# mfathulkr/MA-CJD-Cooperative-Jamming-Decision-Making-via-MARL

Measured on AMD Instinct MI355X. Metric: env-steps/sec (all GPUs; batch_envs=4096/GPU, 3j/4r), higher is better.
Workload: dtype f64; 1 GPU; 3 jammers / 4 radars, batch_envs=4096 per GPU, GRU hidden=64; mode=train, hidden=64, train_batch_episodes=32, updates_per_graph=20, hip_graphs=True, gemm_tuning=True, update=paired: Q-head launches as one grid, mixers as one grid, the chain on one queue, replay_capacity_episodes=8192, mixer_dtype=fp32, mixer=one MFMA launch per direction (f32)

## Files before the change

### include/macjd_nets.h

```cpp
#ifndef MACJD_NETS_H
#define MACJD_NETS_H

#include <stdint.h>

#ifdef __cplusplus
extern "C" {
#endif

typedef struct macjd_qhead_io {
    int64_t n_rows;
    int32_t H, A, n_agents, greedy_only;
    const float* base;  int64_t base_ld;
    const float* P_all; int64_t p_ld;
    const float* W1;    int64_t w1_ld;
    const float* w2;
    const float* b2;
    float* Q;           int64_t q_ld;
    const void* avail;  int32_t avail_elem_size, reserved;
    int64_t av_se, av_sj, av_sa;
    float epsilon;      float reserved2;
    uint64_t seed, counter;
    const float* eps_dev;
    const uint64_t* counter_dev;
    int32_t* T_out32;
// ... 234 lines not shown
    float* sn; float* xhat;
    float* act;
    const float* gy;
    float* gq;
    float* gout1;
    float* g_w1raw;
    float* g_wfraw;
    float* g_v;
} macjd_mixerf_io;

int macjd_mixer_fused_supported(int32_t J, int32_t S, int32_t Hh, int32_t Em);
int macjd_mixer_fused_forward(const macjd_mixerf_io* io, void* hip_stream);
int macjd_mixer_fused_forward_pair(const macjd_mixerf_io* saved, const macjd_mixerf_io* plain, void* hip_stream);
int macjd_mixer_fused_backward(const macjd_mixerf_io* io, void* hip_stream);
int macjd_mixer_fused_backward_td(const macjd_mixerf_io* io, const macjd_tdloss_io* td, const float* tot_m, void* hip_stream);

typedef struct macjd_agent_episode_io {
    int64_t n_envs;
    int32_t T, J, H, A;
    int32_t greedy_only, reserved;
    const float* gi;    int64_t gi_ld;
    const float* P_all; int64_t p_ld;
    const float* h0;
    const float* w_hh;  const float* b_hh;
    const float* W1;    int64_t w1_ld;
    const float* b1;    const float* w2; const float* b2;
    const void* avail;  int32_t avail_elem_size, reserved2;
    int64_t av_se, av_sj, av_sa;
    const float* eps;
    uint64_t seed;
// ... 31 lines not shown
```

### ma-cjd-cooperative-jamming-decision-making-via-marl_amd/_native.py

```python
from __future__ import annotations

import ctypes
import os
from typing import Optional

_PKG_DIR = os.path.dirname(os.path.abspath(__file__))
LIB_NAME = "libmacjd_hip.so"
LIB_PATH = os.environ.get("MACJD_LIB") or os.path.join(_PKG_DIR, LIB_NAME)

ABI_VERSION = 3
STEP_ARITH_F64 = 1
STEP_LANE_KERNEL = 2
STEP_SLOT_KERNEL = 4

EXPORTS = [
    "macjd_abi_version", "macjd_last_error", "macjd_reload_options", "macjd_device_count",
    "macjd_scenario_create", "macjd_scenario_destroy", "macjd_scenario_dims", "macjd_scenario_is_regular",
    "macjd_env_reset", "macjd_env_step", "macjd_env_step_timed",
    "macjd_qhead_select", "macjd_gru_sequence", "macjd_mixer_tail_forward", "macjd_mixer_tail_backward",
    "macjd_mlp_forward", "macjd_mlp_forward_pair", "macjd_td_loss", "macjd_clip_adam_step", "macjd_clip_adam_step_sample", "macjd_clip_adam_step_ln", "macjd_sample_episodes", "macjd_gather_rows",
    "macjd_linear_wgrad", "macjd_linear_wgrad_workspace_floats", "macjd_linear_wgrad_many", "macjd_qhead_input", "macjd_layernorm_forward", "macjd_layernorm_param_grad", "macjd_gru_gates", "macjd_rowdot", "macjd_splitrelu_backward",
    "macjd_mixer_fused_supported", "macjd_mixer_fused_forward", "macjd_mixer_fused_backward", "macjd_mixer_fused_backward_td", "macjd_td_mask_sum",
    "macjd_agent_episode_supported", "macjd_agent_episode", "macjd_env_step_many", "macjd_env_step_many_timed",
    "macjd_qhead_double_q_supported", "macjd_qhead_double_q", "macjd_qhead_taken_supported", "macjd_qhead_taken",
    "macjd_qheads_pair", "macjd_mixer_fused_forward_pair",
]


class NativeLibraryError(RuntimeError):
    pass


class StepIO(ctypes.Structure):
    _fields_ = [
        ("n_envs", ctypes.c_int64), ("env_offset", ctypes.c_int64), ("seed", ctypes.c_uint64),
        ("flags", ctypes.c_uint32), ("reserved", ctypes.c_uint32),
        ("T", ctypes.c_void_p), ("T_se", ctypes.c_int64), ("T_sx", ctypes.c_int64),
        ("P32", ctypes.c_void_p), ("P64", ctypes.c_void_p), ("P_se", ctypes.c_int64), ("P_sx", ctypes.c_int64),
        ("u", ctypes.c_void_p), ("u_se", ctypes.c_int64), ("u_sx", ctypes.c_int64),
        ("episode", ctypes.c_void_p),
# ... 268 lines not shown
    lib.macjd_agent_episode_supported.argtypes = [ctypes.c_int32] * 3
    lib.macjd_agent_episode.restype = ctypes.c_int
    lib.macjd_agent_episode.argtypes = [ctypes.POINTER(AgentEpisodeIO), ctypes.c_void_p]
    lib.macjd_env_step_many.restype = ctypes.c_int
    lib.macjd_env_step_many.argtypes = [ctypes.c_void_p, ctypes.POINTER(StepIO), ctypes.c_int32, ctypes.c_int64, ctypes.c_void_p]
    lib.macjd_env_step_many_timed.restype = ctypes.c_int
    lib.macjd_env_step_many_timed.argtypes = [ctypes.c_void_p, ctypes.POINTER(StepIO), ctypes.c_int32, ctypes.c_int64, ctypes.c_int,
                                              ctypes.c_void_p, ctypes.POINTER(ctypes.c_float)]
    lib.macjd_mixer_fused_supported.restype = ctypes.c_int
    lib.macjd_mixer_fused_supported.argtypes = [ctypes.c_int32] * 4
    for name in ("macjd_mixer_fused_forward", "macjd_mixer_fused_backward"):
        getattr(lib, name).restype = ctypes.c_int
        getattr(lib, name).argtypes = [ctypes.POINTER(MixerFusedIO), ctypes.c_void_p]
    lib.macjd_mixer_fused_backward_td.restype = ctypes.c_int
    lib.macjd_mixer_fused_backward_td.argtypes = [ctypes.POINTER(MixerFusedIO), ctypes.POINTER(TdLossIO), ctypes.c_void_p, ctypes.c_void_p]
    lib.macjd_td_mask_sum.restype = ctypes.c_int
    lib.macjd_td_mask_sum.argtypes = [ctypes.POINTER(TdLossIO), ctypes.c_void_p, ctypes.c_void_p]
    lib.macjd_qhead_taken_supported.restype = ctypes.c_int
    lib.macjd_qhead_taken_supported.argtypes = [ctypes.c_int32, ctypes.c_int32]
    lib.macjd_qhead_taken.restype = ctypes.c_int
    lib.macjd_qhead_taken.argtypes = [ctypes.POINTER(QtakenIO), ctypes.c_void_p]
    lib.macjd_qheads_pair.restype = ctypes.c_int
    lib.macjd_qheads_pair.argtypes = [ctypes.POINTER(QtakenIO), ctypes.POINTER(DoubleQIO), ctypes.c_void_p]
    lib.macjd_mixer_fused_forward_pair.restype = ctypes.c_int
    lib.macjd_mixer_fused_forward_pair.argtypes = [ctypes.POINTER(MixerFusedIO), ctypes.POINTER(MixerFusedIO), ctypes.c_void_p]
    lib.macjd_qhead_input.restype = ctypes.c_int
    lib.macjd_qhead_input.argtypes = [ctypes.POINTER(QinputIO), ctypes.c_void_p]
    lib.macjd_layernorm_forward.restype = ctypes.c_int
    lib.macjd_layernorm_forward.argtypes = [ctypes.POINTER(LayerNormIO), ctypes.c_void_p]
    lib.macjd_gru_gates.restype = ctypes.c_int
# ... 72 lines not shown
```

### ma-cjd-cooperative-jamming-decision-making-via-marl_amd/core/networks.py

```python
from __future__ import annotations

import os

import numpy as np
import torch
import torch.nn as nn
import torch.nn.functional as F

from .. import ops


class RNNAgent(nn.Module):

    def __init__(self, input_shape, args):
        super().__init__()
        self.args = args
        self.n_actions = args.n_actions
        self.input_shape = input_shape
        self.rnn_hidden_dim = args.rnn_hidden_dim
        self.actor_input_dim = input_shape
        self.actor_hidden_dim = args.actor_hidden_dim
        self.actor_output_dim = self.n_actions
        self.actor = nn.Sequential(
            nn.Linear(self.actor_input_dim, self.actor_hidden_dim), nn.ReLU(),
# ... 192 lines not shown
            return self._cat_cache
        ps = self.first_layer_params()
        return torch.cat([p.detach() for p in ps[:4]], dim=0), torch.cat([p.detach() for p in ps[4:]])

    def _forward_fused(self, agent_qs, states):
        q = agent_qs.reshape(-1, self.n_agents)
        s = states.reshape(-1, self.state_dim)
        ln, w_cat_b = self.state_norm, self._first_layer_cat()
        l2 = (self.hyper_w_1[2].weight, self.hyper_w_1[2].bias, self.hyper_w_final[2].weight, self.hyper_w_final[2].bias,
              self.V[2].weight, self.V[2].bias)
        if torch.is_grad_enabled() and (q.requires_grad or ln.weight.requires_grad or l2[0].requires_grad):
            return ops.mixer_fused(q, s, ln.weight, ln.bias, ln.eps, w_cat_b[0], w_cat_b[1], *l2, self.first_layer_params())
        params = ops._mixerf_params(ln.weight, ln.bias, ln.eps, w_cat_b[0], w_cat_b[1], *l2)
        return ops.mixer_fused_forward(q, s, params, save=False)[0]

    def forward_paired_with_next_fused(self, agent_qs, states):
        q = agent_qs.reshape(-1, self.n_agents)
        s = states.reshape(-1, self.state_dim)
        ln, w_cat_b = self.state_norm, self._first_layer_cat()
        params = ops._mixerf_params(ln.weight, ln.bias, ln.eps, w_cat_b[0], w_cat_b[1], self.hyper_w_1[2].weight,
                                    self.hyper_w_1[2].bias, self.hyper_w_final[2].weight, self.hyper_w_final[2].bias,
                                    self.V[2].weight, self.V[2].bias)
        y = ops.pair_mixer_forward_with_next_fused(q, s, params)
        q_tot = y.view(agent_qs.size(0), -1, 1)
        return q_tot.squeeze(1) if q_tot.shape[1] == 1 else q_tot

    def forward(self, agent_qs, states, hyper=None):
        batch_size = agent_qs.size(0)
        if hyper is None and self.fused_available(agent_qs):
            y = self._forward_fused(agent_qs, states)
            q_tot = y.view(batch_size, -1, 1)
            return q_tot.squeeze(1) if q_tot.shape[1] == 1 else q_tot
        raw = hyper if hyper is not None else self.hyper_outputs(states)
        q = agent_qs.reshape(-1, self.n_agents)
        y = ops.mixer_tail(q, *raw)
        q_tot = y.view(batch_size, -1, 1)
        if q_tot.shape[1] == 1:
# ... 3 lines not shown
```

### ma-cjd-cooperative-jamming-decision-making-via-marl_amd/core/qmix.py

```python
from __future__ import annotations

import copy
import os

import numpy as np
import torch
import torch.nn.functional as F
import torch.optim as optim

from .. import hipgraph, ops, options
from .networks import QMixer


def _to(x, dtype, device):
    if isinstance(x, torch.Tensor):
        return x.to(device=device, dtype=dtype)
    return torch.as_tensor(np.asarray(x), device=device).to(dtype)


class QMixLearner:
    def __init__(self, mac, args):
        self.args = args
        self.mac = mac
        self.n_agents = args.n_agents
# ... 278 lines not shown
                validate=False).view(B, T1, J)
            return self.eval_qmix_net(q_taken, st["state"])

        two_streams = dev.type == "cuda" and options.get("UPDATE_STREAMS") != "1"
        target_beside_head = (two_streams and prefetched is not None and fused_dq and pre_actor is not None
                              and self.target_qmix_net.fused_available(st["state"]))
        paired_heads = target_beside_head and self._paired_heads_ok(st, T)
        if paired_heads:
            origin = torch.cuda.current_stream(dev)
            side_work = None
            fork_at = torch.cuda.Event()
            if after_join is not None:
                side_work = lambda: after_join(fork_at)
            if prefetched[1] is not None:
                origin.wait_event(prefetched[1])
            with torch.no_grad():
                bases = scan_chain()
                p_eval = pre_actor[1]
                params = [p_eval if shared else pre_actor[0], p_eval]
                for t_ in list(bases) + [p for p in params if p is not None]:
                    t_.record_stream(origin)
                tq_agents = double_q(bases, params, paired=True)
            q_taken = self.mac.agent.get_q_value_for_action(
                st["hidden_state"].view(n, H), st["actions_discrete"].view(n, 1), st["actions_continuous"].view(n, 1),
                validate=False).view(B, T1, J)
            if after_join is not None:
                fork_at.record(origin)
            with torch.no_grad():
                target_q_tot = self.target_qmix_net.forward_paired_with_next_fused(tq_agents, st["state"])
            eval_q_tot = self.eval_qmix_net(q_taken, st["state"])
            ops.assert_pairs_launched()
            return self._finish_update(st, T, eval_q_tot, target_q_tot, tot_m=prefetched[2] if len(prefetched) > 2 else None,
                                       side_work=side_work, sums_in_backward=True)
        elif target_beside_head:
            origin = torch.cuda.current_stream(dev)
            ts = self._target_stream
            ts.wait_stream(origin)
            with torch.cuda.stream(ts), torch.no_grad():
                bases = scan_chain()
                p_eval = pre_actor[1]
                params = [p_eval if shared else pre_actor[0], p_eval]
                target_q_tot = self.target_qmix_net(double_q(bases, params), st["state"])
                target_done = torch.cuda.Event()
                target_done.record(ts)
            if after_join is not None:
                after_join(False)
            origin.wait_event(prefetched[0])
            eval_q_tot = eval_forward()
# ... 43 lines not shown
                hyper = None if self.target_qmix_net.fused_available(st["state"]) else self.target_qmix_net.hyper_outputs(st["state"])
                target_q_tot = self.target_qmix_net(double_q(bases, params), st["state"], hyper=hyper)
            eval_q_tot = eval_forward()
        return self._finish_update(st, T, eval_q_tot, target_q_tot)

    def _paired_heads_ok(self, st, T):
        B, T1 = st["state"].shape[0], T + 1
        J, H, A = self.n_agents, self.args.rnn_hidden_dim, self.n_actions
        n = B * T1 * J
        head = self.mac.agent.fc2_q_head
        return (st["state"].is_cuda and options.get("UPDATE_STREAMS") != "1" and options.on("PAIRED_HEADS")
                and ops.qhead_double_q_fused_supported(st["obs"].reshape(n, -1), H, A)
                and self.target_qmix_net.fused_available(st["state"]) and self.eval_qmix_net.fused_available(st["state"])
                and ops.qhead_taken_supported(st["hidden_state"].view(n, H), head[0].weight, head[2].weight, A))

    def _finish_update(self, st, T, eval_q_tot, target_q_tot, tot_m=None, side_work=None, sums_in_backward=False):
        for p in self.params:
            p.grad = None
        if eval_q_tot.is_cuda:
            stats_done = stats_branch = None
            if tot_m is not None and ops.fused_mixer_backward_will_run(eval_q_tot):
                origin = torch.cuda.current_stream(eval_q_tot.device)
                ts = self._target_stream
                head_done = torch.cuda.Event()
                if not sums_in_backward:
                    head_done.record(origin)

                def stats_branch():
                    with torch.cuda.stream(ts):
                        ts.wait_event(head_done)
                        out = ops.td_loss_and_grad(eval_q_tot, target_q_tot, st["reward"], st["terminated"], st["filled"],
                                                   self.args.gamma, T - 1, 1)
                        done = torch.cuda.Event()
                        done.record(ts)
                    return out, done

# ... 2 lines not shown
                else:
                    row = self._last_stats4 = torch.empty(4, dtype=torch.float32, device=eval_q_tot.device)
                    loss, eval_mean, target_mean = row[0], row[1], row[2]
                gy = ops.td_grad_in_mixer_backward(eval_q_tot, target_q_tot, st["reward"], st["terminated"], st["filled"],
                                                   self.args.gamma, T - 1, 1, tot_m, stats_row=row if sums_in_backward else None)
            else:
                loss, eval_mean, target_mean, gy, self._last_stats4 = ops.td_loss_and_grad(
                    eval_q_tot, target_q_tot, st["reward"], st["terminated"], st["filled"], self.args.gamma, T - 1, 1)
            hold = self._flat_param is not None and self._world_size() <= 1 and options.on("LN_IN_SQNORM")
            with ops.deferred_wgrad(grad_dst=getattr(self, "_grad_dst", None), hold_lnparam=hold) as dw:
                eval_q_tot.backward(gy)
            assert ops._PENDING_TD is None, "the fused mixer's backward did not take the TD loss's inputs"
            self._held_ln = dw.held
            if side_work is not None:
                side_work()
            if stats_done is not None:
                torch.cuda.current_stream(eval_q_tot.device).wait_event(stats_done)
                for t_ in (self._last_stats4,):
                    t_.record_stream(torch.cuda.current_stream(eval_q_tot.device))
        else:
            loss, eval_mean, target_mean = ops.td_loss_full(eval_q_tot, target_q_tot, st["reward"], st["terminated"],
                                                            st["filled"], self.args.gamma, T - 1, 1)
            loss.backward()
        if self._world_size() > 1 or self._flat_param is not None:
            self._flatten_grads()
        return loss.detach(), eval_mean.detach(), target_mean.detach()

    def _clip_and_step(self, sample_next=None):
        if self._flat_param is not None:
            g = self.optimizer.param_groups[0]
# ... 398 lines not shown
```

### ma-cjd-cooperative-jamming-decision-making-via-marl_amd/csrc/macjd_mixer.hip

```cpp
#include <hip/hip_runtime.h>
#include <math.h>
#include <stdint.h>

#include "../../include/macjd.h"
#include "../../include/macjd_nets.h"
#include "macjd_err.h"
#include "macjd_tdloss.h"

namespace macjd {

typedef float f32x4 __attribute__((ext_vector_type(4)));
typedef float f32x4_u __attribute__((ext_vector_type(4), aligned(4)));

#ifndef MACJD_MX_ABLATE
#define MACJD_MX_ABLATE 0
#endif
constexpr int MX_ABL = MACJD_MX_ABLATE;
constexpr int MX_HH = 128, MX_EM = 64;
constexpr int MX_N1 = 2 * MX_HH + 2 * MX_EM;
constexpr int MX_RELU = 2 * MX_HH + MX_EM;
constexpr int MX_LDH = MX_N1 + 8;
constexpr int MX_KQ2 = MX_HH / 16;

__device__ __forceinline__ float mx_clamp(float x, float lo, float hi) { return fminf(fmaxf(x, lo), hi); }
// ... 52 lines not shown
    const float* hv = Hs + li * MX_LDH + 2 * MX_HH + 16 * g;
#pragma unroll
    for (int k = 0; k < 16; ++k) s = fmaf(hv[k], wv[k], s);
    s += __shfl_xor(s, 16, 64);
    s += __shfl_xor(s, 32, 64);
    return s + bV2;
}

template <int SQ>
struct MixerFwdLds {
    alignas(16) float As[16 * (16 * SQ + 8)];
    alignas(16) float Hs[16 * MX_LDH];
    float part[4][16];
};

template <int J, int SQ, bool SAVE, bool LATE2 = false>
__device__ __forceinline__ void mixer_fused_forward_body(const macjd_mixerf_io& io, const int blk, MixerFwdLds<SQ>& L) {
    constexpr int LDA = 16 * SQ + 8;
    constexpr int T1W = MX_N1 / 16 / 4;
    auto& As = L.As;
    auto& Hs = L.Hs;
    auto& part = L.part;
    const int lane = threadIdx.x & 63;
    const int wave = __builtin_amdgcn_readfirstlane(threadIdx.x >> 6);
    const int li = lane & 15, g = lane >> 4;
    const int64_t m0 = (int64_t)blk * 16;
    const int S = io.S;

    float x[SQ], lnw[SQ], lnb[SQ];
    {
        const int64_t m = m0 + 4 * wave + g;
#pragma unroll
        for (int c = 0; c < SQ; ++c) {
            const int col = li + 16 * c, cc = col < S ? col : S - 1;
            x[c] = (MX_ABL & 8) ? (float)col : io.s[(m < io.M ? m : io.M - 1) * io.s_ld + cc];
            lnw[c] = io.ln_w[cc];
            lnb[c] = io.ln_b[cc];
        }
    }
    float b1v[T1W], b2e[J], wv[16];
#pragma unroll
// ... 88 lines not shown
    const int e = 16 * wave + li;
#pragma unroll
    for (int r = 0; r < 4; ++r) {
        const int row = 4 * g + r;
        float hid = mx_clamp(Hs[row * MX_LDH + MX_RELU + e], -5.0f, 5.0f);
#pragma unroll
        for (int j = 0; j < J; ++j) hid = fmaf(qv[r][j], mx_clamp(acc2[j][r] + b2e[j], 0.0f, 5.0f), hid);
        const float h = hid > 0.0f ? hid : expm1f(hid);
        const float t = mx_sum16(h * mx_clamp(accf[r] + bfe, 0.0f, 5.0f));
        if (li == 0) part[wave][row] = t;
    }
    const float v_raw = (wave == 0) ? mx_v_raw(Hs, wv, bV2, li, g) : 0.0f;
    __syncthreads();
    if (wave == 0 && g == 0) {
        const int64_t m = m0 + li;
        if (m < io.M) io.y[m] = ((part[0][li] + part[1][li]) + (part[2][li] + part[3][li])) + mx_clamp(v_raw, -5.0f, 5.0f);
    }
}

template <int J, int SQ, bool SAVE>
__global__ void __launch_bounds__(256) mixer_fused_forward_kernel(const macjd_mixerf_io io) {
    __shared__ MixerFwdLds<SQ> L;
    mixer_fused_forward_body<J, SQ, SAVE>(io, blockIdx.x, L);
}

template <int J, int SQ>
__global__ void __launch_bounds__(256, (J <= 3) ? 2 : 1) mixer_fused_forward_pair_kernel(const macjd_mixerf_io io_a, const macjd_mixerf_io io_b) {
    __shared__ MixerFwdLds<SQ> L;
    if (blockIdx.y == 0) mixer_fused_forward_body<J, SQ, true, (J <= 3)>(io_a, blockIdx.x, L);
    else mixer_fused_forward_body<J, SQ, false, (J <= 3)>(io_b, blockIdx.x, L);
}

template <int J, bool TD = false>
__global__ void __launch_bounds__(256) mixer_fused_backward_kernel(const macjd_mixerf_io io, const macjd_tdloss_io td,
                                                                    const float* __restrict__ tot_m) {
    constexpr int LDG = J * MX_EM + 8;
    constexpr int LDF = MX_EM + 8;
    constexpr int KQ1 = J * MX_EM / 16;
    constexpr int KQF = MX_EM / 16;
    __shared__ __attribute__((aligned(16))) float Hs[16 * MX_LDH];
    __shared__ __attribute__((aligned(16))) float G1[16 * LDG];
    __shared__ __attribute__((aligned(16))) float Gf[16 * LDF];
    __shared__ float gq_part[4][16][J];
    __shared__ float gv_s[16];
    const int lane = threadIdx.x & 63;
// ... 146 lines not shown
                const int row = 4 * g + r;
                const int64_t m = m0 + row;
                if (m < io.M) {
                    io.gout1[m * MX_N1 + n] = (Hs[row * MX_LDH + n] > 0.0f) ? a1[tt][r] : 0.0f;
                    io.gout1[m * MX_N1 + MX_HH + n] = (Hs[row * MX_LDH + MX_HH + n] > 0.0f) ? af[tt][r] : 0.0f;
                }
            }
        }
    }
#pragma unroll
    for (int i = 0; i < 16 * MX_EM / 256; ++i) {
        const int idx = threadIdx.x + 256 * i;
        const int row = idx / MX_EM, k = idx - row * MX_EM;
        if (m0 + row < io.M)
            io.gout1[(m0 + row) * MX_N1 + 2 * MX_HH + k] = (Hs[row * MX_LDH + 2 * MX_HH + k] > 0.0f) ? gv_s[row] * wvo[i] : 0.0f;
    }
}

template <int PJ>
__device__ __forceinline__ void mx_load_pass(f32x4 (&dst)[PJ][MX_KQ2], const float* __restrict__ W2, int j0, int wave, int li, int g) {
#pragma unroll
    for (int jj = 0; jj < PJ; ++jj) mx_load_frags<MX_KQ2, false>(dst[jj], W2, MX_HH, (j0 + jj) * MX_EM + 16 * wave + li, g);
}

template <int PJ>
__device__ __forceinline__ void mx_pass_tiles(const float* __restrict__ Hs, const f32x4 (&B2)[PJ][MX_KQ2], f32x4 (&acc2)[PJ],
                                              int li, int g) {
#pragma unroll
    for (int j = 0; j < PJ; ++j) acc2[j] = f32x4{0.f, 0.f, 0.f, 0.f};
    const float* a1p = Hs + li * MX_LDH + 4 * g;
// ... 495 lines not shown
    if (!td || !tot_m || td->B < 1 || td->Tm1 < 1 || !td->y || !td->tq || !td->reward || !td->terminated || !td->filled)
        return set_err(MACJD_EINVAL, "%s", "macjd_mixer_fused_backward_td: bad TD-loss argument");
    if (td->gy_cols < td->Tm1 || (int64_t)td->B * td->gy_cols != io->M || td->y_sb < td->Tm1 || td->tq_sb < td->Tm1)
        return set_err(MACJD_EINVAL, "%s", "macjd_mixer_fused_backward_td: rows must be B x gy_cols with gy_cols >= Tm1");
    if (io->M == 0) return MACJD_OK;
    const dim3 grid((unsigned)((io->M + 15) / 16) + (td->stats ? 1u : 0u)), block(256);
    hipStream_t s = (hipStream_t)hip_stream;
    if (io->J == 2) hipLaunchKernelGGL((mixer_fused_backward_kernel<2, true>), grid, block, 0, s, *io, *td, tot_m);
    else if (io->J == 3) hipLaunchKernelGGL((mixer_fused_backward_kernel<3, true>), grid, block, 0, s, *io, *td, tot_m);
    else if (io->J == 6) hipLaunchKernelGGL((mixer_fused_backward_kernel<6, true>), grid, block, 0, s, *io, *td, tot_m);
    else hipLaunchKernelGGL((mixer_fused_backward_wide_kernel<12, 4, true>), grid, block, 0, s, *io, *td, tot_m);
    const hipError_t err = hipGetLastError();
    if (err != hipSuccess) return set_err(MACJD_EDEVICE, "macjd_mixer_fused_backward_td: %s", hipGetErrorString(err));
    return MACJD_OK;
}
```

### ma-cjd-cooperative-jamming-decision-making-via-marl_amd/ops.py

```python
from __future__ import annotations

import ctypes
import os
from typing import Optional, Tuple

import numpy as np
import torch
import torch.nn.functional as F

from . import _native, options


def _stream(t: torch.Tensor) -> int:
    return torch.cuda.current_stream(t.device).cuda_stream


def _f32c(t: torch.Tensor) -> torch.Tensor:
    if t.dtype != torch.float32:
        t = t.float()
    return t if t.stride(-1) == 1 else t.contiguous()


def _qhead_fill(io: _native.QheadIO, base, P_all, W1, w2, b2, H: int, A: int, n_agents: int):
    io.n_rows, io.H, io.A, io.n_agents = base.shape[0], H, A, n_agents
# ... 90 lines not shown
        keep += [b1, w2, b2]
        setattr(io, f"W1_{tag}", W1.data_ptr()); setattr(io, f"w1{tag}_ld", W1.stride(0))
        setattr(io, f"b1_{tag}", b1.data_ptr()); setattr(io, f"w2_{tag}", w2.data_ptr()); setattr(io, f"b2_{tag}", b2.data_ptr())
    out = torch.empty(N, dtype=torch.float32, device=h_e.device)
    io.out = out.data_ptr()
    am = None
    if want_argmax:
        am = torch.empty(N, dtype=torch.int64, device=h_e.device)
        io.argmax_out = am.data_ptr()
    keep += [P_e, P_t]
    return io, keep, out, am


_PAIRED_DQ = None
_PAIRED_MIXER = None


def pair_double_q_with_next_taken(h_eval, P_eval, head_eval, h_tgt, P_tgt, head_tgt, H: int, A: int, p_row_map=None):
    global _PAIRED_DQ
    assert _PAIRED_DQ is None, "a paired Double-DQN launch is already waiting"
    io, keep, out, _ = _doubleq_io(h_eval, P_eval, head_eval, h_tgt, P_tgt, head_tgt, H, A, False, p_row_map)
    _PAIRED_DQ = (io, keep, out)
    return out


def pair_mixer_forward_with_next_fused(q, s, params):
    global _PAIRED_MIXER
    assert _PAIRED_MIXER is None, "a paired mixer launch is already waiting"
    q, s = q.detach().float().contiguous(), _f32c(s.detach())
    y = torch.empty((s.shape[0], 1), dtype=torch.float32, device=q.device)
    io = _mixerf_io(q, s, params)
    io.y = y.data_ptr()
    _PAIRED_MIXER = (io, (q, s, params), y)
    return y


def assert_pairs_launched():
    global _PAIRED_DQ, _PAIRED_MIXER
    left = [n for n, v in (("Double-DQN", _PAIRED_DQ), ("mixer", _PAIRED_MIXER)) if v is not None]
    _PAIRED_DQ = _PAIRED_MIXER = None
    if left:
        raise RuntimeError("paired launch not taken by the autograd forward it was meant for: " + ", ".join(left))


def qhead_select(base, P_all, W1, w2, b2, H: int, A: int, n_agents: int, avail: Optional[torch.Tensor],
                 epsilon: float, greedy_only: bool, seed: int, counter: int, want_q: bool = False,
                 eps_dev: Optional[torch.Tensor] = None, counter_dev: Optional[torch.Tensor] = None,
                 out_T32: Optional[torch.Tensor] = None, out_P: Optional[torch.Tensor] = None
                 ) -> Tuple[torch.Tensor, torch.Tensor, torch.Tensor, Optional[torch.Tensor]]:
    if not base.is_cuda:
        raise RuntimeError("qhead_select is the HIP path; host tensors use the selector in utils.action_selectors")
    lib = _native.load()
    N = base.shape[0]
    E = N // n_agents
    dev = base.device
# ... 327 lines not shown
        pair, _PAIRED_MIXER = _PAIRED_MIXER, None
    with torch.cuda.device(q.device):
        if pair is not None:
            _native.check(lib.macjd_mixer_fused_forward_pair(ctypes.byref(io), ctypes.byref(pair[0]), _stream(q)),
                          "macjd_mixer_fused_forward_pair")
        else:
            _native.check(lib.macjd_mixer_fused_forward(ctypes.byref(io), _stream(q)), "macjd_mixer_fused_forward")
    return y, q, saved


class _FusedMixer(torch.autograd.Function):

    @staticmethod
    def forward(ctx, q, s, ln_w, ln_b, eps, w_cat, b_cat, W2, b2, Wf2, bf2, wV2, bV2, *first):
        params = _mixerf_params(ln_w, ln_b, eps, w_cat, b_cat, W2, b2, Wf2, bf2, wV2, bV2)
        y, qc, (sn, xhat, act) = mixer_fused_forward(q, s, params, save=True)
        ctx.save_for_backward(qc, sn, xhat, act, w_cat, W2, Wf2, wV2, ln_w, ln_b, b2, bf2, bV2)
        ctx.params = {k: v for k, v in params.items() if k in ("eps",)}
        ctx.sizes = [p.shape[0] for p in first[:len(first) // 2]]
        ctx.keys = {"b_cat": grad_key(b_cat), "ln_w": grad_key(ln_w), "ln_b": grad_key(ln_b), "b2": grad_key(b2),
                    "bf2": grad_key(bf2), "bV2": grad_key(bV2)}
        ctx.n_first = len(first)
        return y

    @staticmethod
    def backward(ctx, gy):
        lib = _native.load()
        q, sn, xhat, act, w_cat, W2, Wf2, wV2, ln_w, ln_b, b2, bf2, bV2 = ctx.saved_tensors
        M, J = q.shape
        Hh, Em = W2.shape[1], Wf2.shape[0]
        dev = q.device
        gy = gy.detach().float().contiguous()
        gq = torch.empty((M, J), dtype=torch.float32, device=dev)
        gout1 = torch.empty((M, 2 * Hh + 2 * Em), dtype=torch.float32, device=dev)
        g_w1 = torch.empty((M, J * Em), dtype=torch.float32, device=dev)
        g_wf = torch.empty((M, Em), dtype=torch.float32, device=dev)
        g_v = torch.empty((M, 1), dtype=torch.float32, device=dev)
        params = _mixerf_params(ln_w, ln_b, ctx.params["eps"], w_cat, gout1[0], W2, b2, Wf2, bf2, wV2, bV2)
        io = _mixerf_io(q, None, params)
        io.act, io.gy, io.gq, io.gout1 = act.data_ptr(), gy.data_ptr(), gq.data_ptr(), gout1.data_ptr()
        io.g_w1raw, io.g_wfraw, io.g_v = g_w1.data_ptr(), g_wf.data_ptr(), g_v.data_ptr()
        global _PENDING_TD
        pend, _PENDING_TD = _PENDING_TD, None
        with torch.cuda.device(dev):
            if pend is not None:
                assert pend[2] == M, "td_grad_in_mixer_backward: the loss rows are not this mixer's rows"
                _native.check(lib.macjd_mixer_fused_backward_td(ctypes.byref(io), ctypes.byref(pend[0]), pend[3].data_ptr(),
                                                                _stream(q)), "macjd_mixer_fused_backward_td")
            else:
                _native.check(lib.macjd_mixer_fused_backward(ctypes.byref(io), _stream(q)), "macjd_mixer_fused_backward")
        nd = ctx.needs_input_grad
        gW1, gb1 = linear_wgrad(gout1, sn, want_bias=True, w_key=grad_key(w_cat), b_key=ctx.keys["b_cat"])
        G, _ = linear_wgrad(gout1, xhat, want_bias=False)
        gW2, gb2 = linear_wgrad(g_w1, act[:, :Hh], want_bias=True, w_key=grad_key(W2), b_key=ctx.keys["b2"], need=(nd[7], nd[8]))
        gWf, gbf = linear_wgrad(g_wf, act[:, Hh:2 * Hh], want_bias=True, w_key=grad_key(Wf2), b_key=ctx.keys["bf2"], need=(nd[9], nd[10]))
        gWv, gbv = linear_wgrad(g_v, act[:, 2 * Hh:2 * Hh + Em], want_bias=True, w_key=grad_key(wV2), b_key=ctx.keys["bV2"],
                                need=(nd[11], nd[12]))
        K = w_cat.shape[1]
        dgamma, dbeta = _grad_dst(ctx.keys["ln_w"], (K,)), _grad_dst(ctx.keys["ln_b"], (K,))
        if dgamma is None:
            dgamma = torch.empty(K, dtype=torch.float32, device=dev)
        if dbeta is None:
            dbeta = torch.empty(K, dtype=torch.float32, device=dev)
        lio = _native.LnParamIO()
        lio.C, lio.K = w_cat.shape[0], K
        lio.W, lio.w_ld, lio.G, lio.g_ld = w_cat.data_ptr(), w_cat.stride(0), G.data_ptr(), G.stride(0)
        lio.gb, lio.dgamma, lio.dbeta = gb1.data_ptr(), dgamma.data_ptr(), dbeta.data_ptr()
        stream = _stream(q)

        def post(lio=lio, keep=(G, w_cat), dev=dev, stream=stream):
            with torch.cuda.device(dev):
                _native.check(_native.load().macjd_layernorm_param_grad(ctypes.byref(lio), stream), "macjd_layernorm_param_grad")

        post.lnparam = lio
        if _DEFERRED_WGRAD is not None:
            _DEFERRED_POST.append(post)
        else:
            post()
        first = tuple(gW1.split(ctx.sizes, 0)) + tuple(gb1.split(ctx.sizes, 0))
        return (gq, None, dgamma, dbeta, None, None, None, gW2, gb2, gWf, gbf, gWv, gbv) + first


def mixer_fused(q, s, ln_w, ln_b, eps, w_cat, b_cat, W2, b2, Wf2, bf2, wV2, bV2, first_params):
    return _FusedMixer.apply(q, s, ln_w, ln_b, eps, w_cat, b_cat, W2, b2, Wf2, bf2, wV2, bV2, *first_params)


def enable_gemm_tuning(results_file: Optional[str] = None, max_tuning_ms: int = 30) -> bool:
    try:
        import torch.cuda.tunable as tunable
        tunable.enable(True)
        tunable.tuning_enable(True)
        tunable.set_max_tuning_duration(int(max_tuning_ms))
        if results_file:
            tunable.set_filename(results_file)
        return True
# ... 805 lines not shown
```

### ma-cjd-cooperative-jamming-decision-making-via-marl_amd/options.py

```python
from __future__ import annotations

import os

_DEFAULTS = {
    "UPDATE_STREAMS": "2", "UPDATES_PER_GRAPH": "1", "PIPELINED_GROUP": "1", "SHARED_BODY": "1",
    "LEARNER_STATIC_OBS": "1", "ACTOR_IN_SCAN": "1", "DEVICE_SAMPLER": "1", "LN_IN_SQNORM": "1", "WGRAD_OUTER": "1",
    "QHEAD_TAKEN": "1", "PAIRED_HEADS": "1", "GRAPHED_ALLREDUCE": "0",
}
_values = None


def reload() -> None:
    global _values
    _values = {k: os.environ.get("MACJD_" + k, d) for k, d in _DEFAULTS.items()}


def get(name: str) -> str:
    if _values is None:
        reload()
    return _values[name]


def on(name: str) -> bool:
    return get(name) != "0"
# ... 1 lines not shown
```

Baseline: 32.84 million env-steps/s.

## Fuse eval and target mixer forward, TD loss and mixer backward into one kernel

Adds a mixer training kernel with 512 threads per block. One half runs the eval mixer forward and the other half runs the target mixer forward on the next-step rows. The eval half then computes the TD-loss gradient and the mixer backward in the same block, reusing forward accumulators kept in registers. This removes separate forward, TD and backward launches and the global round-trips for y and gy. The loss statistics move to a side stream, computed late. The cost is higher register and LDS pressure per block and a more complex placeholder-based autograd handoff.

```diff
diff --git a/include/macjd_nets.h b/include/macjd_nets.h
--- a/include/macjd_nets.h
+++ b/include/macjd_nets.h
@@ -272,6 +272,8 @@
 int macjd_mixer_fused_forward_pair(const macjd_mixerf_io* saved, const macjd_mixerf_io* plain, void* hip_stream);
 int macjd_mixer_fused_backward(const macjd_mixerf_io* io, void* hip_stream);
 int macjd_mixer_fused_backward_td(const macjd_mixerf_io* io, const macjd_tdloss_io* td, const float* tot_m, void* hip_stream);
+int macjd_mixer_fused_train(const macjd_mixerf_io* eval, const macjd_mixerf_io* target, const macjd_tdloss_io* td,
+                            const float* tot_m, void* hip_stream);
 
 typedef struct macjd_agent_episode_io {
     int64_t n_envs;
diff --git a/ma-cjd-cooperative-jamming-decision-making-via-marl_amd/_native.py b/ma-cjd-cooperative-jamming-decision-making-via-marl_amd/_native.py
--- a/ma-cjd-cooperative-jamming-decision-making-via-marl_amd/_native.py
+++ b/ma-cjd-cooperative-jamming-decision-making-via-marl_amd/_native.py
@@ -23,7 +23,7 @@
     "macjd_mixer_fused_supported", "macjd_mixer_fused_forward", "macjd_mixer_fused_backward", "macjd_mixer_fused_backward_td", "macjd_td_mask_sum",
     "macjd_agent_episode_supported", "macjd_agent_episode", "macjd_env_step_many", "macjd_env_step_many_timed",
     "macjd_qhead_double_q_supported", "macjd_qhead_double_q", "macjd_qhead_taken_supported", "macjd_qhead_taken",
-    "macjd_qheads_pair", "macjd_mixer_fused_forward_pair",
+    "macjd_qheads_pair", "macjd_mixer_fused_forward_pair", "macjd_mixer_fused_train",
 ]
 
 
@@ -322,6 +322,9 @@
         getattr(lib, name).argtypes = [ctypes.POINTER(MixerFusedIO), ctypes.c_void_p]
     lib.macjd_mixer_fused_backward_td.restype = ctypes.c_int
     lib.macjd_mixer_fused_backward_td.argtypes = [ctypes.POINTER(MixerFusedIO), ctypes.POINTER(TdLossIO), ctypes.c_void_p, ctypes.c_void_p]
+    lib.macjd_mixer_fused_train.restype = ctypes.c_int
+    lib.macjd_mixer_fused_train.argtypes = [ctypes.POINTER(MixerFusedIO), ctypes.POINTER(MixerFusedIO), ctypes.POINTER(TdLossIO),
+                                            ctypes.c_void_p, ctypes.c_void_p]
     lib.macjd_td_mask_sum.restype = ctypes.c_int
     lib.macjd_td_mask_sum.argtypes = [ctypes.POINTER(TdLossIO), ctypes.c_void_p, ctypes.c_void_p]
     lib.macjd_qhead_taken_supported.restype = ctypes.c_int
diff --git a/ma-cjd-cooperative-jamming-decision-making-via-marl_amd/core/networks.py b/ma-cjd-cooperative-jamming-decision-making-via-marl_amd/core/networks.py
--- a/ma-cjd-cooperative-jamming-decision-making-via-marl_amd/core/networks.py
+++ b/ma-cjd-cooperative-jamming-decision-making-via-marl_amd/core/networks.py
@@ -230,13 +230,16 @@
         params = ops._mixerf_params(ln.weight, ln.bias, ln.eps, w_cat_b[0], w_cat_b[1], *l2)
         return ops.mixer_fused_forward(q, s, params, save=False)[0]
 
-    def forward_paired_with_next_fused(self, agent_qs, states):
+    def forward_paired_with_next_fused(self, agent_qs, states, td=None):
         q = agent_qs.reshape(-1, self.n_agents)
         s = states.reshape(-1, self.state_dim)
         ln, w_cat_b = self.state_norm, self._first_layer_cat()
         params = ops._mixerf_params(ln.weight, ln.bias, ln.eps, w_cat_b[0], w_cat_b[1], self.hyper_w_1[2].weight,
                                     self.hyper_w_1[2].bias, self.hyper_w_final[2].weight, self.hyper_w_final[2].bias,
                                     self.V[2].weight, self.V[2].bias)
+        if td is not None:
+            y, placeholder = ops.pair_mixer_train_with_next_fused(q, s, params, **td)
+            return y.view(agent_qs.size(0), -1, 1), placeholder
         y = ops.pair_mixer_forward_with_next_fused(q, s, params)
         q_tot = y.view(agent_qs.size(0), -1, 1)
         return q_tot.squeeze(1) if q_tot.shape[1] == 1 else q_tot
diff --git a/ma-cjd-cooperative-jamming-decision-making-via-marl_amd/core/qmix.py b/ma-cjd-cooperative-jamming-decision-making-via-marl_amd/core/qmix.py
--- a/ma-cjd-cooperative-jamming-decision-making-via-marl_amd/core/qmix.py
+++ b/ma-cjd-cooperative-jamming-decision-making-via-marl_amd/core/qmix.py
@@ -316,24 +316,35 @@
                 side_work = lambda: after_join(fork_at)
             if prefetched[1] is not None:
                 origin.wait_event(prefetched[1])
-            with torch.no_grad():
-                bases = scan_chain()
-                p_eval = pre_actor[1]
-                params = [p_eval if shared else pre_actor[0], p_eval]
-                for t_ in list(bases) + [p for p in params if p is not None]:
-                    t_.record_stream(origin)
-                tq_agents = double_q(bases, params, paired=True)
-            q_taken = self.mac.agent.get_q_value_for_action(
-                st["hidden_state"].view(n, H), st["actions_discrete"].view(n, 1), st["actions_continuous"].view(n, 1),
-                validate=False).view(B, T1, J)
-            if after_join is not None:
-                fork_at.record(origin)
-            with torch.no_grad():
-                target_q_tot = self.target_qmix_net.forward_paired_with_next_fused(tq_agents, st["state"])
-            eval_q_tot = self.eval_qmix_net(q_taken, st["state"])
-            ops.assert_pairs_launched()
-            return self._finish_update(st, T, eval_q_tot, target_q_tot, tot_m=prefetched[2] if len(prefetched) > 2 else None,
-                                       side_work=side_work, sums_in_backward=True)
+            tot_m = prefetched[2] if len(prefetched) > 2 else None
+            mixer_train = tot_m is not None and options.on("MIXER_TRAIN") and J in (2, 3)
+            train_gy = None
+            try:
+                with torch.no_grad():
+                    bases = scan_chain()
+                    p_eval = pre_actor[1]
+                    params = [p_eval if shared else pre_actor[0], p_eval]
+                    for t_ in list(bases) + [p for p in params if p is not None]:
+                        t_.record_stream(origin)
+                    tq_agents = double_q(bases, params, paired=True)
+                q_taken = self.mac.agent.get_q_value_for_action(
+                    st["hidden_state"].view(n, H), st["actions_discrete"].view(n, 1), st["actions_continuous"].view(n, 1),
+                    validate=False).view(B, T1, J)
+                if after_join is not None:
+                    fork_at.record(origin)
+                with torch.no_grad():
+                    if mixer_train:
+                        target_q_tot, train_gy = self.target_qmix_net.forward_paired_with_next_fused(
+                            tq_agents, st["state"], td=dict(reward=st["reward"], terminated=st["terminated"], filled=st["filled"],
+                                                            gamma=self.args.gamma, Tm1=T - 1, tot_m=tot_m))
+                    else:
+                        target_q_tot = self.target_qmix_net.forward_paired_with_next_fused(tq_agents, st["state"])
+                eval_q_tot = self.eval_qmix_net(q_taken, st["state"])
+                ops.assert_pairs_launched()
+            finally:
+                ops.clear_pending_pairs()
+            return self._finish_update(st, T, eval_q_tot, target_q_tot, tot_m=tot_m, side_work=side_work, sums_in_backward=True,
+                                       train_gy=train_gy)
         elif target_beside_head:
             origin = torch.cuda.current_stream(dev)
             ts = self._target_stream
@@ -407,12 +418,29 @@
                 and self.target_qmix_net.fused_available(st["state"]) and self.eval_qmix_net.fused_available(st["state"])
                 and ops.qhead_taken_supported(st["hidden_state"].view(n, H), head[0].weight, head[2].weight, A))
 
-    def _finish_update(self, st, T, eval_q_tot, target_q_tot, tot_m=None, side_work=None, sums_in_backward=False):
+    def _finish_update(self, st, T, eval_q_tot, target_q_tot, tot_m=None, side_work=None, sums_in_backward=False,
+                       train_gy=None):
         for p in self.params:
             p.grad = None
         if eval_q_tot.is_cuda:
-            stats_done = stats_branch = None
-            if tot_m is not None and ops.fused_mixer_backward_will_run(eval_q_tot):
+            stats_done = stats_branch = sums_late = None
+            if train_gy is not None:
+                origin = torch.cuda.current_stream(eval_q_tot.device)
+                ts = self._target_stream
+                head_done = torch.cuda.Event()
+                head_done.record(origin)
+                row = self._last_stats4 = torch.empty(4, dtype=torch.float32, device=eval_q_tot.device)
+                loss, eval_mean, target_mean = row[0], row[1], row[2]
+                gy = train_gy
+
+                def sums_late():
+                    ts.wait_event(head_done)
+                    with torch.cuda.stream(ts):
+                        ops.td_loss_sums_into(row, eval_q_tot, target_q_tot, st["reward"], st["terminated"], st["filled"],
+                                              self.args.gamma, T - 1, 1)
+                    for t_ in (row, eval_q_tot, target_q_tot):
+                        t_.record_stream(ts)
+            elif tot_m is not None and ops.fused_mixer_backward_will_run(eval_q_tot):
                 origin = torch.cuda.current_stream(eval_q_tot.device)
                 ts = self._target_stream
                 head_done = torch.cuda.Event()
@@ -445,6 +473,8 @@
             self._held_ln = dw.held
             if side_work is not None:
                 side_work()
+            if sums_late is not None:
+                sums_late()
             if stats_done is not None:
                 torch.cuda.current_stream(eval_q_tot.device).wait_event(stats_done)
                 for t_ in (self._last_stats4,):
diff --git a/ma-cjd-cooperative-jamming-decision-making-via-marl_amd/csrc/macjd_mixer.hip b/ma-cjd-cooperative-jamming-decision-making-via-marl_amd/csrc/macjd_mixer.hip
--- a/ma-cjd-cooperative-jamming-decision-making-via-marl_amd/csrc/macjd_mixer.hip
+++ b/ma-cjd-cooperative-jamming-decision-making-via-marl_amd/csrc/macjd_mixer.hip
@@ -90,17 +90,22 @@
     float part[4][16];
 };
 
-template <int J, int SQ, bool SAVE, bool LATE2 = false>
-__device__ __forceinline__ void mixer_fused_forward_body(const macjd_mixerf_io& io, const int blk, MixerFwdLds<SQ>& L) {
+template <int J>
+struct MixerKeep {
+    f32x4 acc2[J], accf;
+    float qv[4][J], b2e[J], bfe, v_raw, y;
+};
+
+template <int J, int SQ, bool SAVE, bool LATE2 = false, bool KEEP = false>
+__device__ __forceinline__ void mixer_fused_forward_body(const macjd_mixerf_io& io, const int64_t m0, const int wave,
+                                                         MixerFwdLds<SQ>& L, MixerKeep<J>* keep = nullptr) {
     constexpr int LDA = 16 * SQ + 8;
     constexpr int T1W = MX_N1 / 16 / 4;
     auto& As = L.As;
     auto& Hs = L.Hs;
     auto& part = L.part;
     const int lane = threadIdx.x & 63;
-    const int wave = __builtin_amdgcn_readfirstlane(threadIdx.x >> 6);
     const int li = lane & 15, g = lane >> 4;
-    const int64_t m0 = (int64_t)blk * 16;
     const int S = io.S;
 
     float x[SQ], lnw[SQ], lnb[SQ];
@@ -219,21 +224,37 @@
     __syncthreads();
     if (wave == 0 && g == 0) {
         const int64_t m = m0 + li;
-        if (m < io.M) io.y[m] = ((part[0][li] + part[1][li]) + (part[2][li] + part[3][li])) + mx_clamp(v_raw, -5.0f, 5.0f);
+        const float y = ((part[0][li] + part[1][li]) + (part[2][li] + part[3][li])) + mx_clamp(v_raw, -5.0f, 5.0f);
+        if (m < io.M) io.y[m] = y;
+        if (KEEP) keep->y = y;
+    }
+    if (KEEP) {
+#pragma unroll
+        for (int j = 0; j < J; ++j) {
+            keep->acc2[j] = acc2[j];
+            keep->b2e[j] = b2e[j];
+#pragma unroll
+            for (int r = 0; r < 4; ++r) keep->qv[r][j] = qv[r][j];
+        }
+        keep->accf = accf;
+        keep->bfe = bfe;
+        keep->v_raw = v_raw;
     }
 }
 
 template <int J, int SQ, bool SAVE>
 __global__ void __launch_bounds__(256) mixer_fused_forward_kernel(const macjd_mixerf_io io) {
     __shared__ MixerFwdLds<SQ> L;
-    mixer_fused_forward_body<J, SQ, SAVE>(io, blockIdx.x, L);
+    mixer_fused_forward_body<J, SQ, SAVE>(io, (int64_t)blockIdx.x * 16, __builtin_amdgcn_readfirstlane(threadIdx.x >> 6), L);
 }
 
 template <int J, int SQ>
 __global__ void __launch_bounds__(256, (J <= 3) ? 2 : 1) mixer_fused_forward_pair_kernel(const macjd_mixerf_io io_a, const macjd_mixerf_io io_b) {
     __shared__ MixerFwdLds<SQ> L;
-    if (blockIdx.y == 0) mixer_fused_forward_body<J, SQ, true, (J <= 3)>(io_a, blockIdx.x, L);
-    else mixer_fused_forward_body<J, SQ, false, (J <= 3)>(io_b, blockIdx.x, L);
+    const int64_t m0 = (int64_t)blockIdx.x * 16;
+    const int wave = __builtin_amdgcn_readfirstlane(threadIdx.x >> 6);
+    if (blockIdx.y == 0) mixer_fused_forward_body<J, SQ, true, (J <= 3)>(io_a, m0, wave, L);
+    else mixer_fused_forward_body<J, SQ, false, (J <= 3)>(io_b, m0, wave, L);
 }
 
 template <int J, bool TD = false>
@@ -410,6 +431,166 @@
         const int row = idx / MX_EM, k = idx - row * MX_EM;
         if (m0 + row < io.M)
             io.gout1[(m0 + row) * MX_N1 + 2 * MX_HH + k] = (Hs[row * MX_LDH + 2 * MX_HH + k] > 0.0f) ? gv_s[row] * wvo[i] : 0.0f;
+    }
+}
+
+template <int J>
+struct MixerTrainLds {
+    MixerFwdLds<J> ev, tg;
+    alignas(16) float G1[16 * (J * MX_EM + 8)];
+    alignas(16) float Gf[16 * (MX_EM + 8)];
+    float gq_part[4][16][J];
+    float gv_s[16];
+    float ys[16], tqs[16];
+};
+
+template <int J>
+__global__ void __launch_bounds__(512) mixer_fused_train_kernel(const macjd_mixerf_io io, const macjd_mixerf_io tio,
+                                                                 const macjd_tdloss_io td, const float* __restrict__ tot_m) {
+    constexpr int LDG = J * MX_EM + 8;
+    constexpr int LDF = MX_EM + 8;
+    constexpr int KQ1 = J * MX_EM / 16;
+    constexpr int KQF = MX_EM / 16;
+    __shared__ MixerTrainLds<J> L;
+    const int lane = threadIdx.x & 63;
+    const int wave8 = __builtin_amdgcn_readfirstlane(threadIdx.x >> 6);
+    const int wave = wave8 & 3;
+    const bool eval_half = wave8 < 4;
+    const int li = lane & 15, g = lane >> 4;
+    const int64_t m0 = (int64_t)blockIdx.x * 16;
+    const float* Hs = L.ev.Hs;
+
+    float rw[5], term[5], mk[5];
+    bool live[5];
+    if (eval_half) {
+#pragma unroll
+        for (int r = 0; r < 5; ++r) {
+            const int row = r < 4 ? 4 * g + r : li;
+            const int64_t mc = (m0 + row < io.M) ? m0 + row : io.M - 1;
+            const int cols = (int)td.gy_cols;
+            const int b = (int)(mc / cols), t = (int)(mc - (int64_t)b * cols);
+            const int tc = t < td.Tm1 ? t : td.Tm1 - 1;
+            term[r] = td.terminated[b * td.t_sb + tc * td.t_st] ? 1.0f : 0.0f;
+            mk[r] = td.filled[b * td.f_sb + tc * td.f_st] ? 1.0f : 0.0f;
+            rw[r] = td.reward[b * td.r_sb + tc * td.r_st];
+            live[r] = t < td.Tm1;
+        }
+    }
+
+    MixerKeep<J> K;
+    f32x4 D1[KQ1], Df[KQF];
+    if (eval_half) {
+        mixer_fused_forward_body<J, J, true, true, true>(io, m0, wave, L.ev, &K);
+        if (wave == 0 && g == 0) L.ys[li] = K.y;
+    } else {
+        MixerKeep<J> Kt;
+        mixer_fused_forward_body<J, J, false, true, true>(tio, m0 + 1, wave, L.tg, &Kt);
+        if (wave == 0 && g == 0) L.tqs[li] = Kt.y;
+    }
+    {
+        const int n = 16 * wave8 + li;
+#pragma unroll
+        for (int Q = 0; Q < KQ1; ++Q)
+#pragma unroll
+            for (int jj = 0; jj < 4; ++jj) D1[Q][jj] = io.W2[(int64_t)(16 * Q + 4 * g + jj) * MX_HH + n];
+#pragma unroll
+        for (int Q = 0; Q < KQF; ++Q)
+#pragma unroll
+            for (int jj = 0; jj < 4; ++jj) Df[Q][jj] = io.Wf2[(int64_t)(16 * Q + 4 * g + jj) * MX_HH + n];
+    }
+    float wvo[2];
+#pragma unroll
+    for (int i = 0; i < 2; ++i) wvo[i] = io.wV2[(threadIdx.x + 512 * i) & (MX_EM - 1)];
+    __syncthreads();
+
+    if (eval_half) {
+        const float scale = 2.0f / tot_m[0];
+        float gyv[5];
+#pragma unroll
+        for (int r = 0; r < 5; ++r) {
+            const int row = r < 4 ? 4 * g + r : li;
+            const float target = rw[r] + td.gamma * (1.0f - term[r]) * L.tqs[row];
+            const float gv = scale * mk[r] * (L.ys[row] - target);
+            gyv[r] = live[r] ? gv : 0.0f;
+        }
+        const int e = 16 * wave + li;
+#pragma unroll
+        for (int r = 0; r < 4; ++r) {
+            const int row = 4 * g + r;
+            const int64_t m = m0 + row;
+            const float b1r = Hs[row * MX_LDH + MX_RELU + e];
+            float hid = mx_clamp(b1r, -5.0f, 5.0f);
+            float w1r[J];
+#pragma unroll
+            for (int j = 0; j < J; ++j) {
+                w1r[j] = K.acc2[j][r] + K.b2e[j];
+                hid = fmaf(K.qv[r][j], mx_clamp(w1r[j], 0.0f, 5.0f), hid);
+            }
+            const float h = hid > 0.0f ? hid : expm1f(hid);
+            const float wfr = K.accf[r] + K.bfe;
+            const float ghid = gyv[r] * mx_clamp(wfr, 0.0f, 5.0f) * (hid > 0.0f ? 1.0f : h + 1.0f);
+            const float gwf = (wfr >= 0.0f && wfr <= 5.0f) ? gyv[r] * h : 0.0f;
+            const float gb1 = (b1r >= -5.0f && b1r <= 5.0f) ? ghid : 0.0f;
+            L.Gf[row * LDF + e] = gwf;
+            if (m < io.M) {
+                io.g_wfraw[m * MX_EM + e] = gwf;
+                io.gout1[m * MX_N1 + MX_RELU + e] = gb1;
+            }
+#pragma unroll
+            for (int j = 0; j < J; ++j) {
+                const float gw = (w1r[j] >= 0.0f && w1r[j] <= 5.0f) ? ghid * K.qv[r][j] : 0.0f;
+                L.G1[row * LDG + j * MX_EM + e] = gw;
+                if (m < io.M) io.g_w1raw[m * (J * MX_EM) + j * MX_EM + e] = gw;
+                const float t = mx_sum16(ghid * mx_clamp(w1r[j], 0.0f, 5.0f));
+                if (li == 0) L.gq_part[wave][row][j] = t;
+            }
+        }
+        if (wave == 0 && g == 0) {
+            const int64_t m = m0 + li;
+            const float gv = (K.v_raw >= -5.0f && K.v_raw <= 5.0f) ? gyv[4] : 0.0f;
+            L.gv_s[li] = gv;
+            if (m < io.M) io.g_v[m] = gv;
+        }
+    }
+    __syncthreads();
+    if (threadIdx.x < 16 * J) {
+        const int row = threadIdx.x / J, j = threadIdx.x - row * J;
+        if (m0 + row < io.M)
+            io.gq[(m0 + row) * J + j] = (L.gq_part[0][row][j] + L.gq_part[1][row][j]) + (L.gq_part[2][row][j] + L.gq_part[3][row][j]);
+    }
+    {
+        f32x4 a1 = f32x4{0.f, 0.f, 0.f, 0.f}, af = f32x4{0.f, 0.f, 0.f, 0.f};
+        const float* gp = L.G1 + li * LDG + 4 * g;
+        const float* fp = L.Gf + li * LDF + 4 * g;
+#pragma unroll
+        for (int Q = 0; Q < KQ1; ++Q) {
+            const f32x4 a = *reinterpret_cast<const f32x4*>(gp + 16 * Q);
+#pragma unroll
+            for (int jj = 0; jj < 4; ++jj) a1 = __builtin_amdgcn_mfma_f32_16x16x4f32(a[jj], D1[Q][jj], a1, 0, 0, 0);
+        }
+#pragma unroll
+        for (int Q = 0; Q < KQF; ++Q) {
+            const f32x4 a = *reinterpret_cast<const f32x4*>(fp + 16 * Q);
+#pragma unroll
+            for (int jj = 0; jj < 4; ++jj) af = __builtin_amdgcn_mfma_f32_16x16x4f32(a[jj], Df[Q][jj], af, 0, 0, 0);
+        }
+        const int n = 16 * wave8 + li;
+#pragma unroll
+        for (int r = 0; r < 4; ++r) {
+            const int row = 4 * g + r;
+            const int64_t m = m0 + row;
+            if (m < io.M) {
+                io.gout1[m * MX_N1 + n] = (Hs[row * MX_LDH + n] > 0.0f) ? a1[r] : 0.0f;
+                io.gout1[m * MX_N1 + MX_HH + n] = (Hs[row * MX_LDH + MX_HH + n] > 0.0f) ? af[r] : 0.0f;
+            }
+        }
+    }
+#pragma unroll
+    for (int i = 0; i < 16 * MX_EM / 512; ++i) {
+        const int idx = threadIdx.x + 512 * i;
+        const int row = idx / MX_EM, k = idx - row * MX_EM;
+        if (m0 + row < io.M)
+            io.gout1[(m0 + row) * MX_N1 + 2 * MX_HH + k] = (Hs[row * MX_LDH + 2 * MX_HH + k] > 0.0f) ? L.gv_s[row] * wvo[i] : 0.0f;
     }
 }
 
@@ -935,3 +1116,32 @@
     if (err != hipSuccess) return set_err(MACJD_EDEVICE, "macjd_mixer_fused_backward_td: %s", hipGetErrorString(err));
     return MACJD_OK;
 }
+
+extern "C" int macjd_mixer_fused_train(const macjd_mixerf_io* eval, const macjd_mixerf_io* target, const macjd_tdloss_io* td,
+                                       const float* tot_m, void* hip_stream) {
+    using namespace macjd;
+    int rc = mixerf_check(eval, false);
+    if (rc != MACJD_OK) return rc;
+    rc = mixerf_check(eval, true, true);
+    if (rc != MACJD_OK) return rc;
+    rc = mixerf_check(target, false);
+    if (rc != MACJD_OK) return rc;
+    if (!eval->save || target->save) return set_err(MACJD_EINVAL, "%s", "macjd_mixer_fused_train: the eval mixer saves, the target mixer does not");
+    if (eval->J != target->J || eval->S != target->S || eval->M != target->M)
+        return set_err(MACJD_EINVAL, "%s", "macjd_mixer_fused_train: the two mixers differ in J / S / M");
+    if (eval->J != 2 && eval->J != 3) return set_err(MACJD_EINVAL, "%s", "macjd_mixer_fused_train: J must be 2 or 3");
+    if (!td || !tot_m || td->B < 1 || td->Tm1 < 1 || !td->y || !td->tq || !td->reward || !td->terminated || !td->filled)
+        return set_err(MACJD_EINVAL, "%s", "macjd_mixer_fused_train: bad TD-loss argument");
+    if (td->gy_cols < td->Tm1 + 1 || (int64_t)td->B * td->gy_cols != eval->M)
+        return set_err(MACJD_EINVAL, "%s", "macjd_mixer_fused_train: rows must be B x gy_cols with gy_cols > Tm1");
+    if (td->y != eval->y || td->y_sb != td->gy_cols || td->tq != target->y + 1 || td->tq_sb != td->gy_cols)
+        return set_err(MACJD_EINVAL, "%s", "macjd_mixer_fused_train: td->y / td->tq must be eval->y / target->y + 1 with row pitch gy_cols");
+    if (eval->M == 0) return MACJD_OK;
+    const dim3 grid((unsigned)((eval->M + 15) / 16)), block(512);
+    hipStream_t s = (hipStream_t)hip_stream;
+    if (eval->J == 2) hipLaunchKernelGGL((mixer_fused_train_kernel<2>), grid, block, 0, s, *eval, *target, *td, tot_m);
+    else hipLaunchKernelGGL((mixer_fused_train_kernel<3>), grid, block, 0, s, *eval, *target, *td, tot_m);
+    const hipError_t err = hipGetLastError();
+    if (err != hipSuccess) return set_err(MACJD_EDEVICE, "macjd_mixer_fused_train: %s", hipGetErrorString(err));
+    return MACJD_OK;
+}
diff --git a/ma-cjd-cooperative-jamming-decision-making-via-marl_amd/ops.py b/ma-cjd-cooperative-jamming-decision-making-via-marl_amd/ops.py
--- a/ma-cjd-cooperative-jamming-decision-making-via-marl_amd/ops.py
+++ b/ma-cjd-cooperative-jamming-decision-making-via-marl_amd/ops.py
@@ -128,6 +128,7 @@
 
 _PAIRED_DQ = None
 _PAIRED_MIXER = None
+_PAIRED_TRAIN = None
 
 
 def pair_double_q_with_next_taken(h_eval, P_eval, head_eval, h_tgt, P_tgt, head_tgt, H: int, A: int, p_row_map=None):
@@ -149,10 +150,39 @@
     return y
 
 
+def pair_mixer_train_with_next_fused(q, s, params, reward, terminated, filled, gamma, Tm1, tot_m):
+    global _PAIRED_TRAIN
+    assert _PAIRED_TRAIN is None and _PAIRED_MIXER is None, "a paired mixer launch is already waiting"
+    q, s = q.detach().float().contiguous(), _f32c(s.detach())
+    M = s.shape[0]
+    B = reward.shape[0]
+    assert M % B == 0 and M // B > int(Tm1), "pair_mixer_train_with_next_fused: rows must be B x T1 with T1 > Tm1"
+    T1 = M // B
+    y = torch.empty((M, 1), dtype=torch.float32, device=q.device)
+    io = _mixerf_io(q, s, params)
+    io.y = y.data_ptr()
+    td = _native.TdLossIO()
+    td.B, td.Tm1, td.gamma = B, int(Tm1), float(gamma)
+    td.y_sb = T1
+    td.tq, td.tq_sb = y.data_ptr() + 4, T1
+    td.gy, td.gy_sb, td.gy_cols = None, T1, T1
+    td.reward, td.r_sb, td.r_st = reward.data_ptr(), reward.stride(0), reward.stride(1)
+    td.terminated, td.t_sb, td.t_st = terminated.data_ptr(), terminated.stride(0), terminated.stride(1)
+    td.filled, td.f_sb, td.f_st = filled.data_ptr(), filled.stride(0), filled.stride(1)
+    placeholder = torch.empty((B, T1, 1), dtype=torch.float32, device=q.device)
+    _PAIRED_TRAIN = (io, td, (q, s, params, reward, terminated, filled, tot_m, y), placeholder)
+    return y, placeholder
+
+
+def clear_pending_pairs():
+    global _PAIRED_DQ, _PAIRED_MIXER, _PAIRED_TRAIN
+    _PAIRED_DQ = _PAIRED_MIXER = _PAIRED_TRAIN = None
+
+
 def assert_pairs_launched():
-    global _PAIRED_DQ, _PAIRED_MIXER
-    left = [n for n, v in (("Double-DQN", _PAIRED_DQ), ("mixer", _PAIRED_MIXER)) if v is not None]
-    _PAIRED_DQ = _PAIRED_MIXER = None
+    left = [n for n, v in (("Double-DQN", _PAIRED_DQ), ("mixer", _PAIRED_MIXER), ("mixer training", _PAIRED_TRAIN))
+            if v is not None]
+    clear_pending_pairs()
     if left:
         raise RuntimeError("paired launch not taken by the autograd forward it was meant for: " + ", ".join(left))
 
@@ -510,7 +540,13 @@
     @staticmethod
     def forward(ctx, q, s, ln_w, ln_b, eps, w_cat, b_cat, W2, b2, Wf2, bf2, wV2, bV2, *first):
         params = _mixerf_params(ln_w, ln_b, eps, w_cat, b_cat, W2, b2, Wf2, bf2, wV2, bV2)
-        y, qc, (sn, xhat, act) = mixer_fused_forward(q, s, params, save=True)
+        global _PAIRED_TRAIN
+        train, _PAIRED_TRAIN = _PAIRED_TRAIN, None
+        ctx.train = None
+        if train is not None:
+            y, qc, (sn, xhat, act), ctx.train = _mixer_train(q, s, params, train)
+        else:
+            y, qc, (sn, xhat, act) = mixer_fused_forward(q, s, params, save=True)
         ctx.save_for_backward(qc, sn, xhat, act, w_cat, W2, Wf2, wV2, ln_w, ln_b, b2, bf2, bV2)
         ctx.params = {k: v for k, v in params.items() if k in ("eps",)}
         ctx.sizes = [p.shape[0] for p in first[:len(first) // 2]]
@@ -526,6 +562,10 @@
         M, J = q.shape
         Hh, Em = W2.shape[1], Wf2.shape[0]
         dev = q.device
+        if ctx.train is not None:
+            placeholder, (gq, gout1, g_w1, g_wf, g_v) = ctx.train
+            assert gy.data_ptr() == placeholder.data_ptr(), "mixer training launch: backward not seeded with its placeholder"
+            return _FusedMixer._wgrads(ctx, q, sn, xhat, act, w_cat, W2, Wf2, wV2, ln_w, ln_b, gq, gout1, g_w1, g_wf, g_v)
         gy = gy.detach().float().contiguous()
         gq = torch.empty((M, J), dtype=torch.float32, device=dev)
         gout1 = torch.empty((M, 2 * Hh + 2 * Em), dtype=torch.float32, device=dev)
@@ -545,6 +585,12 @@
                                                                 _stream(q)), "macjd_mixer_fused_backward_td")
             else:
                 _native.check(lib.macjd_mixer_fused_backward(ctypes.byref(io), _stream(q)), "macjd_mixer_fused_backward")
+        return _FusedMixer._wgrads(ctx, q, sn, xhat, act, w_cat, W2, Wf2, wV2, ln_w, ln_b, gq, gout1, g_w1, g_wf, g_v)
+
+    @staticmethod
+    def _wgrads(ctx, q, sn, xhat, act, w_cat, W2, Wf2, wV2, ln_w, ln_b, gq, gout1, g_w1, g_wf, g_v):
+        Hh, Em = W2.shape[1], Wf2.shape[0]
+        dev = q.device
         nd = ctx.needs_input_grad
         gW1, gb1 = linear_wgrad(gout1, sn, want_bias=True, w_key=grad_key(w_cat), b_key=ctx.keys["b_cat"])
         G, _ = linear_wgrad(gout1, xhat, want_bias=False)
@@ -575,6 +621,35 @@
             post()
         first = tuple(gW1.split(ctx.sizes, 0)) + tuple(gb1.split(ctx.sizes, 0))
         return (gq, None, dgamma, dbeta, None, None, None, gW2, gb2, gWf, gbf, gWv, gbv) + first
+
+
+def _mixer_train(q, s, params, train):
+    lib = _native.load()
+    tio, td, keep, placeholder = train
+    q, s = q.detach().float().contiguous(), _f32c(s.detach())
+    M, S = s.shape
+    J, dev = q.shape[1], q.device
+    assert M == tio.M and td.B * td.gy_cols == M, "mixer training launch: the two mixers / the loss differ in rows"
+    y = torch.empty((M, 1), dtype=torch.float32, device=dev)
+    io = _mixerf_io(q, s, params)
+    width = 2 * io.Hh + 2 * io.Em
+    sn = torch.empty((M, S), dtype=torch.float32, device=dev)
+    xhat = torch.empty((M, S), dtype=torch.float32, device=dev)
+    act = torch.empty((M, width), dtype=torch.float32, device=dev)
+    gq = torch.empty((M, J), dtype=torch.float32, device=dev)
+    gout1 = torch.empty((M, width), dtype=torch.float32, device=dev)
+    g_w1 = torch.empty((M, J * io.Em), dtype=torch.float32, device=dev)
+    g_wf = torch.empty((M, io.Em), dtype=torch.float32, device=dev)
+    g_v = torch.empty((M, 1), dtype=torch.float32, device=dev)
+    io.y, io.save, io.sn, io.xhat, io.act = y.data_ptr(), 1, sn.data_ptr(), xhat.data_ptr(), act.data_ptr()
+    io.gq, io.gout1 = gq.data_ptr(), gout1.data_ptr()
+    io.g_w1raw, io.g_wfraw, io.g_v = g_w1.data_ptr(), g_wf.data_ptr(), g_v.data_ptr()
+    td.y = y.data_ptr()
+    tot_m = keep[6]
+    with torch.cuda.device(dev):
+        _native.check(lib.macjd_mixer_fused_train(ctypes.byref(io), ctypes.byref(tio), ctypes.byref(td), tot_m.data_ptr(),
+                                                  _stream(q)), "macjd_mixer_fused_train")
+    return y, q, (sn, xhat, act), (placeholder, (gq, gout1, g_w1, g_wf, g_v))
 
 
 def mixer_fused(q, s, ln_w, ln_b, eps, w_cat, b_cat, W2, b2, Wf2, bf2, wV2, bV2, first_params):
diff --git a/ma-cjd-cooperative-jamming-decision-making-via-marl_amd/options.py b/ma-cjd-cooperative-jamming-decision-making-via-marl_amd/options.py
--- a/ma-cjd-cooperative-jamming-decision-making-via-marl_amd/options.py
+++ b/ma-cjd-cooperative-jamming-decision-making-via-marl_amd/options.py
@@ -5,7 +5,7 @@
 _DEFAULTS = {
     "UPDATE_STREAMS": "2", "UPDATES_PER_GRAPH": "1", "PIPELINED_GROUP": "1", "SHARED_BODY": "1",
     "LEARNER_STATIC_OBS": "1", "ACTOR_IN_SCAN": "1", "DEVICE_SAMPLER": "1", "LN_IN_SQNORM": "1", "WGRAD_OUTER": "1",
-    "QHEAD_TAKEN": "1", "PAIRED_HEADS": "1", "GRAPHED_ALLREDUCE": "0",
+    "QHEAD_TAKEN": "1", "PAIRED_HEADS": "1", "MIXER_TRAIN": "1", "GRAPHED_ALLREDUCE": "0",
 }
 _values = None
 
```

Measured after the change: 33.97 million env-steps/s, median of 6. 1.03x the previous value.
